# jgmarti84/radar-processor

Hardware: AMD Instinct MI355X
Metric: Mvoxels/s gridded (+ achieved HBM GB/s in roofline) (higher is better)
Workload: dtype f32

## Files before the change

### radar_processor_amd/csrc/rg_compact_layout.hpp

```cpp
#pragma once

#include <type_traits>

#include "rg_common.hpp"
#include "rg_row_phase.hpp"

using rg_u32x4 = unsigned __attribute__((ext_vector_type(4)));
__device__ rg_u32x4 rg_buffer_load_v4u32(__amdgpu_buffer_rsrc_t, int voffset, int soffset, int aux)
    __asm("llvm.amdgcn.raw.ptr.buffer.load.v4i32");

__device__ float rg_fmul_legacy(float, float) __asm("llvm.amdgcn.fmul.legacy");

namespace rgl {

struct ChunkGrid {
  long line_len;
  long lines_per_plane;
  long n_planes;
  unsigned nsx;
  unsigned nyg;
  unsigned rot_step;
  unsigned seg_base;
  unsigned seg_extra;
  unsigned grp0;
};

struct RowwiseColumns {
  const int32_t* order = nullptr;
  float* planes = nullptr;
  float* col_val = nullptr;
  int32_t* col_arg = nullptr;
  long n_xy = 0;
  unsigned n_cols = 0;
  int pieces = 1, keep_lo = 0, n_keep = 0, col_lo = 0, col_hi = 0;
};

struct RowwisePlanes : RowwiseColumns {
  float* col_min = nullptr;
  float* col_mean = nullptr;
  const int32_t* sel[RG_MAX_SEL_PLANES] = {};
  float* samples = nullptr;
  int n_sel = 0;
};

struct StreamArgs {
  const void* indptr;
  bool is_i64;
  const void* records;
  const int64_t* rec_ptr;
  int rec_order;
  unsigned w_base;
  const int64_t* dict_ptr;
  const int32_t* dict;
  long n_vox, n_pairs, line_len, lines_per_plane;
  const float* packed;
  int n_fields, stride;
  long n_gates;
  float fill;
  float* out;
  int window_cap;
  int lanes_hint;
  hipStream_t stream;
  int max_fields;
  bool need_out;
  bool need_packed;
  const uint16_t* row_end16 = nullptr;
};

}

namespace {

using rgl::ChunkGrid;
using rgl::StreamArgs;
using rgl::RowwiseColumns;
using rgl::RowwisePlanes;
using rg::f32x2;
using rg::f32x4;
using rsrc_t = __amdgpu_buffer_rsrc_t;
constexpr int kRsrcRaw32 = 0x00020000;

__device__ __forceinline__ rsrc_t make_rsrc(const void* base, long bytes) {
  const unsigned nb = bytes >= 0xFFFFFFFFL ? 0xFFFFFFFFu : bytes <= 0 ? 0u : (unsigned)bytes;
  return __builtin_amdgcn_make_buffer_rsrc(const_cast<void*>(base), 0, (int)nb, kRsrcRaw32);
}

constexpr int kH = RG_COMPACT_LINES;

__device__ __forceinline__ unsigned block_chunk(const ChunkGrid& g, unsigned bid) {
  const unsigned grp = bid / g.nsx;
  const unsigned col = bid - grp * g.nsx;
  const unsigned rot = col + ((grp + g.grp0) * g.rot_step) % g.nsx;
  return grp * g.nsx + (rot >= g.nsx ? rot - g.nsx : rot);
}

__host__ __device__ inline long chunk_count(const ChunkGrid& g) { return g.n_planes * (long)g.nyg * (long)g.nsx; }

struct Segment {
  long r0;
  long seg;
  int nrows;
};

__device__ __forceinline__ Segment chunk_segment(const ChunkGrid& g, unsigned chunk, int w) {
  const unsigned grp = chunk / g.nsx;
  const unsigned sx = chunk - grp * g.nsx;
  const unsigned plane = grp / g.nyg;
  const unsigned yg = grp - plane * g.nyg;
  const long y = (long)yg * kH + w;
  Segment s;
  if (y >= g.lines_per_plane) {
    s.r0 = 0;
    s.seg = 0;
    s.nrows = 0;
    return s;
  }
  s.seg = ((long)plane * g.lines_per_plane + y) * g.nsx + sx;
  const unsigned x0 = sx * g.seg_base + (sx < g.seg_extra ? sx : g.seg_extra);
  s.r0 = ((long)plane * g.lines_per_plane + y) * g.line_len + (long)x0;
  s.nrows = (int)(g.seg_base + (sx < g.seg_extra ? 1u : 0u));
  return s;
}

using rg::stride_for;

constexpr int kDenseMaxDict = RG_DENSE_MAX_DICT;
__host__ __device__ inline bool rec_is_dense(long nd_all) { return nd_all <= kDenseMaxDict; }
__host__ __device__ inline long rec_units(long n_rec, bool dense) { return dense ? (14 * n_rec + 15) >> 4 : n_rec; }

struct RecFields {
  unsigned wc[3];
  unsigned pos[3];
};

template <bool DENSE>
__device__ __forceinline__ RecFields rec_decode(const rg_u32x4& ld, unsigned par) {
  RecFields r;
  if constexpr (DENSE) {
    const unsigned sh = par << 4;
    const unsigned w2 = __builtin_amdgcn_alignbit(ld.w, ld.x, sh);
    r.wc[0] = ld.y;
    r.wc[1] = ld.z;
    r.wc[2] = w2;
    r.pos[0] = __builtin_amdgcn_ubfe(ld.w, sh, 11u);
    const unsigned p1h = __builtin_amdgcn_ubfe(ld.w, sh + 11u, 5u);
    r.pos[1] = __builtin_amdgcn_alignbit(p1h, ld.y, 26);
    r.pos[2] = __builtin_amdgcn_alignbit(w2 >> 26, ld.z, 26);
  } else {
    r.wc[0] = ld.x;
    r.wc[1] = ld.y;
    r.wc[2] = ld.z;
    r.pos[0] = ld.w & 0xFFFFu;
    r.pos[1] = ld.w >> 16;
    unsigned p2b = ld.y >> 26, p2c = ld.z >> 26;
    asm volatile("" : "+v"(p2b), "+v"(p2c));
    r.pos[2] = (p2c << 12) | ((p2b << 6) | (ld.x >> 26));
  }
  return r;
}

__device__ __forceinline__ void rec_encode_dense(const unsigned (&code)[3], const unsigned (&pos)[3], bool odd, unsigned short (&h)[7]) {
  const unsigned m1 = (code[0] & 0x3FFFFFFu) | ((pos[1] & 0x3Fu) << 26);
  const unsigned m2 = (code[1] & 0x3FFFFFFu) | ((pos[2] & 0x3Fu) << 26);
  const unsigned w2 = (code[2] & 0x3FFFFFFu) | (((pos[2] >> 6) & 0x1Fu) << 26);
  const unsigned short p = (unsigned short)((pos[0] & 0x7FFu) | (((pos[1] >> 6) & 0x1Fu) << 11));
  const unsigned short m1l = (unsigned short)m1, m1h = (unsigned short)(m1 >> 16), m2l = (unsigned short)m2,
                       m2h = (unsigned short)(m2 >> 16), w2h = (unsigned short)(w2 >> 16);
  h[0] = (unsigned short)w2;
  h[1] = odd ? m1l : w2h;
  h[2] = odd ? m1h : m1l;
  h[3] = odd ? m2l : m1h;
  h[4] = odd ? m2h : m2l;
  h[5] = odd ? w2h : m2h;
  h[6] = p;
}

bool make_chunk_grid(int64_t n_rows, int64_t line_len, int64_t lines_per_plane, ChunkGrid* cg) {
  if (line_len <= 0) line_len = n_rows > 0 ? n_rows : 1;
  if (n_rows % line_len != 0) return false;
  const long n_lines = n_rows / line_len;
  if (lines_per_plane <= 0) lines_per_plane = n_lines > 0 ? n_lines : 1;
  if (n_lines % lines_per_plane != 0) return false;
  cg->line_len = line_len;
  cg->lines_per_plane = lines_per_plane;
  cg->n_planes = n_lines / lines_per_plane;
  const long nsx = (line_len + 63) / 64, nyg = (lines_per_plane + kH - 1) / kH;
  if (nsx > 0x7FFFFFFFL || nyg > 0x7FFFFFFFL) return false;
  cg->nsx = (unsigned)nsx;
  cg->nyg = (unsigned)nyg;
  cg->seg_base = (unsigned)(line_len / nsx);
  cg->seg_extra = (unsigned)(line_len % nsx);
  cg->rot_step = RG_COMPACT_ROTATION;
  cg->grp0 = 0;
  return true;
}

inline int check_stream_args(const char* fn, const StreamArgs& a, ChunkGrid* cg) {
  RG_REQUIRE(a.rec_order == RG_REC_ORDER_SEGMENT || a.rec_order == RG_REC_ORDER_DISPATCH, RG_EINVAL,
             "%s: rec_order=%d is neither RG_REC_ORDER_SEGMENT nor RG_REC_ORDER_DISPATCH", fn, a.rec_order);
  RG_REQUIRE(a.n_fields >= 1 && a.n_fields <= a.max_fields, RG_EUNSUPPORTED, "%s: n_fields=%d not in 1..%d", fn, a.n_fields,
             a.max_fields);
  RG_REQUIRE(a.stride == stride_for(a.n_fields), RG_EINVAL, "%s: stride=%d, expected %d for %d fields", fn, a.stride,
             stride_for(a.n_fields), a.n_fields);
  RG_REQUIRE(a.indptr && a.dict_ptr && a.rec_ptr && (a.out || !a.need_out), RG_EINVAL, "%s: null indptr/dict_ptr/rec_ptr%s", fn,
             a.need_out ? "/out" : "");
  RG_REQUIRE(a.n_vox >= 0 && a.n_pairs >= 0, RG_EINVAL, "%s: negative size", fn);
  RG_REQUIRE(a.n_pairs == 0 || (a.records && a.dict && a.packed && a.n_gates > 0), RG_EINVAL,
             "%s: pairs present but records/dict/packed/n_gates missing", fn);
  RG_REQUIRE(!a.need_packed || (a.packed && a.n_gates > 0), RG_EINVAL, "%s: packed fields missing", fn);
  RG_REQUIRE(a.n_gates <= 0x7FFFFFFFL, RG_EUNSUPPORTED, "%s: n_gates exceeds int32 gate indices", fn);
  RG_REQUIRE(a.n_vox <= 0x3FFFFFFFFFL, RG_EUNSUPPORTED, "%s: n_vox too large for one launch", fn);
  RG_REQUIRE(a.window_cap >= 0 && a.window_cap <= RG_COMPACT_MAX_WINDOW, RG_EINVAL, "%s: window_cap %d outside 0..%d", fn,
             a.window_cap, RG_COMPACT_MAX_WINDOW);
  RG_REQUIRE(rg::aligned16(a.records), RG_EALIGN, "%s: records must be 16-byte aligned", fn);
  RG_REQUIRE(!a.need_packed || rg::aligned16(a.packed), RG_EALIGN, "%s: packed must be 16-byte aligned", fn);
  RG_REQUIRE((a.w_base & 0x3FFFFFFu) == 0, RG_EINVAL,
             "%s: w_base=0x%08x must have its low 26 bits clear (exponent a multiple of 8)", fn, a.w_base);
  RG_REQUIRE(a.lanes_hint == 0 || (a.lanes_hint >= 1 && a.lanes_hint <= 64 && (a.lanes_hint & (a.lanes_hint - 1)) == 0) ||
                 (a.lanes_hint > 70 && a.lanes_hint <= 99), RG_EINVAL,
             "%s: the lane split must be 0, a power of two up to 64, or 71..99", fn);
  if (a.n_vox == 0) return RG_OK;
  RG_REQUIRE(make_chunk_grid(a.n_vox, a.line_len, a.lines_per_plane, cg), RG_EINVAL,
             "%s: n_vox=%ld is not planes x lines_per_plane=%ld x line_len=%ld", fn, a.n_vox, a.lines_per_plane, a.line_len);
  RG_REQUIRE(chunk_count(*cg) <= 0x7FFFFFFFL, RG_EUNSUPPORTED, "%s: too many chunks for one launch", fn);
  return RG_OK;
}

template <int NF> struct RowwiseConfig;
template <> struct RowwiseConfig<1> { static constexpr int kpre = 3, target = 4; static constexpr bool regs = false; };
template <> struct RowwiseConfig<2> { static constexpr int kpre = 3, target = 4; static constexpr bool regs = false; };
template <> struct RowwiseConfig<3> { static constexpr int kpre = 3, target = 6; static constexpr bool regs = true; };
template <> struct RowwiseConfig<4> { static constexpr int kpre = 3, target = 8; static constexpr bool regs = true; };
template <> struct RowwiseConfig<5> { static constexpr int kpre = 3, target = 8; static constexpr bool regs = true; };
template <> struct RowwiseConfig<6> { static constexpr int kpre = 3, target = 8; static constexpr bool regs = true; };
template <> struct RowwiseConfig<7> { static constexpr int kpre = 3, target = 8; static constexpr bool regs = true; };
template <> struct RowwiseConfig<8> { static constexpr int kpre = 3, target = 12; static constexpr bool regs = true; };

template <int NF> constexpr bool rowwise_bytemask() { return NF >= 3; }
template <int NF> constexpr int rowwise_value_words() {
  return rowwise_bytemask<NF>() ? (NF <= 4 ? 4 : 8) : 2;
}
template <int NF> constexpr int rowwise_mask_words() { return !rowwise_bytemask<NF>() || NF == 3 ? 0 : NF == 4 ? 1 : 2; }
template <int NF> constexpr int rowwise_entry_words() { return rowwise_value_words<NF>() + rowwise_mask_words<NF>(); }


struct ColumnBest {
  float v;
  int idx;
};

__device__ __forceinline__ void column_max_step(ColumnBest& acc, float v, int z) {
  if (acc.idx < 0) {
    if (!isnan(v)) { acc.v = v; acc.idx = z; }
  } else {
    const bool keep = acc.v >= v || isnan(v);
    if (!keep) { acc.v = v; acc.idx = z; }
  }
}

__device__ __forceinline__ void column_min_step(float& acc, float v) {
  const bool keep = acc <= v || isnan(v);
  if (!keep) acc = v;
}

}

int rg_launch_tile_packed(const rgl::StreamArgs& a, const rgl::ChunkGrid& cg);
```

### radar_processor_amd/csrc/rg_csr_rowwise.hpp

```cpp
#pragma once

#include "rg_compact_layout.hpp"

namespace {

constexpr int kRowwiseChunksPerBlock = 1;

#define RG_ROWWISE_BOUNDS __launch_bounds__(64 * kH, (COLS == 2 ? (NF <= 2 ? 5 : 4) : (COLS == 0 && NF >= 4 && NF <= 6) ? 5 : 1))
template <typename IndT, int NF, int STRIDE, int COLS = 0, int REGS = -1>
__global__ RG_ROWWISE_BOUNDS void csr_compact_rowwise_kernel(
    const IndT* __restrict__ indptr, const int64_t* __restrict__ dict_ptr, const int32_t* __restrict__ dict, ChunkGrid cg,
    const float* __restrict__ packed, unsigned last_gate, float fill, int window_cap, long n_vox, float* __restrict__ out,
    const rg_u32x4* __restrict__ rec, const int64_t* __restrict__ rec_ptr, unsigned w_base, int lanes_hint,
    int rec_order, unsigned n_chunks, int chunks_per_block, const std::conditional_t<COLS == 2, RowwisePlanes, RowwiseColumns> cols,
    const uint16_t* __restrict__ row_end16) {
  static_assert(NF >= 1 && NF <= 8 && STRIDE == stride_for(NF), "passes of 1-8 fields");
  constexpr bool PLANES = COLS == 2;
  static_assert(!PLANES || NF <= 4, "the planes mode is the column mode of 1-4 fields");
  using Cfg = RowwiseConfig<NF>;
  constexpr int KPRE = Cfg::kpre;
  constexpr bool kByteMask = rowwise_bytemask<NF>();
  constexpr bool kRegs = REGS < 0 ? Cfg::regs : REGS != 0;
  constexpr bool kScatter = NF >= 5 && !COLS;
  constexpr int kFenceMinNF = 3;
  constexpr bool kPremask = NF == 1;
  extern __shared__ __attribute__((aligned(16))) float window[];
  constexpr int kVW = rowwise_value_words<NF>(), kMW = rowwise_mask_words<NF>();
#if defined(__HIP_DEVICE_COMPILE__) && !defined(__gfx950__)
#error "the byte masks assume v_cvt_pk_f32_fp8 decodes OCP e4m3 (0x38 = 1.0), as on gfx950"
#endif
  constexpr unsigned kMaskOne = 0x38u;
  (void)kMW;
  unsigned* const maskw = reinterpret_cast<unsigned*>(window + (size_t)(window_cap + 1) * kVW);
  __shared__ f32x2 rowacc_all[kRegs ? 1 : kH][kRegs ? 2 : 64 * NF];
  constexpr bool kStage = kScatter;
  __shared__ __attribute__((aligned(16))) float stage_all[kStage ? kH : 1][kStage ? 64 * 8 : 4];

  const int lane = threadIdx.x & 63;
  const int wv = __builtin_amdgcn_readfirstlane(threadIdx.x >> 6);
  f32x2* rowacc = rowacc_all[kRegs ? 0 : wv];
  float* const stage = stage_all[kStage ? wv : 0];
  unsigned wmask = 0x3FFFFFFu;
  asm volatile("" : "+v"(wmask));

  unsigned col_yg = 0, col_sx = 0, col_piece = 0;
  int col_z0 = 0;
  ColumnBest best[COLS ? NF : 1];
  float pmin[PLANES ? NF : 1], psum[PLANES ? NF : 1];
  int pcnt[PLANES ? NF : 1];
  if constexpr (PLANES) {
#pragma unroll
    for (int f = 0; f < NF; ++f) { pmin[f] = __builtin_nanf(""); psum[f] = 0.0f; pcnt[f] = 0; }
  }
  if constexpr (COLS) {
    const unsigned item = cols.order ? (unsigned)cols.order[blockIdx.x] : blockIdx.x;
    col_piece = item / cols.n_cols;
    const unsigned q = item - col_piece * cols.n_cols;
    col_yg = q / cg.nsx;
    const unsigned c = q - col_yg * cg.nsx;
    col_sx = c + (col_yg * cg.rot_step) % cg.nsx;
    col_sx = col_sx >= cg.nsx ? col_sx - cg.nsx : col_sx;
    col_z0 = (int)((long)col_piece * cg.n_planes / cols.pieces);
    chunks_per_block = (int)((long)(col_piece + 1) * cg.n_planes / cols.pieces) - col_z0;
#pragma unroll
    for (int f = 0; f < NF; ++f) { best[f].v = __builtin_nanf(""); best[f].idx = -1; }
  }
  long col_xy = 0;
  int col_nrows = 0;
  const int n_cb = COLS ? chunks_per_block : kRowwiseChunksPerBlock;
  for (int cb = 0; cb < n_cb; ++cb) {
  unsigned bid, chunk;
  if constexpr (COLS) {
    const unsigned grp = (unsigned)(col_z0 + cb) * cg.nyg + col_yg;
    chunk = grp * cg.nsx + col_sx;
    const unsigned shift = ((grp + cg.grp0) * cg.rot_step) % cg.nsx;
    bid = grp * cg.nsx + (col_sx >= shift ? col_sx - shift : col_sx + cg.nsx - shift);
  } else {
    bid = blockIdx.x * (unsigned)kRowwiseChunksPerBlock + (unsigned)cb;
    if (bid >= n_chunks) break;
    chunk = block_chunk(cg, bid);
  }
  if constexpr (!COLS) {
    if (rec_order == RG_REC_ORDER_DISPATCH && rec_ptr[(long)bid * kH] == rec_ptr[((long)bid + 1) * kH]) {
      const Segment se = chunk_segment(cg, chunk, wv);
      if (lane < se.nrows) {
#pragma unroll
        for (int f = 0; f < NF; ++f) out[(size_t)f * n_vox + se.r0 + lane] = fill;
      }
      continue;
    }
  }
  if (cb > 0) __syncthreads();
  float mine_p[NF], mine_w[NF];
#pragma unroll
  for (int f = 0; f < NF; ++f) mine_p[f] = mine_w[f] = 0.0f;

  const long d0 = dict_ptr[chunk];
  const int nd_all = (int)(dict_ptr[chunk + 1] - d0);
  const bool split = nd_all > 65536;
  const bool windowed = nd_all <= window_cap;

  const Segment sg = chunk_segment(cg, chunk, wv);
  const int nrows = sg.nrows;
  const long r0 = sg.r0;
  int span = 0, rs_o = 0, re_o = 0;
  unsigned e16 = RG_ROW_END16_WIDE;
  if (row_end16 && nrows) e16 = row_end16[r0 + (lane < nrows ? lane : nrows - 1)];
  if (__builtin_amdgcn_readlane((int)e16, 63) != (int)RG_ROW_END16_WIDE) {
    re_o = (int)e16;
    rs_o = __builtin_amdgcn_update_dpp(0, (int)e16, 0x138 , 0xF, 0xF, false);
    span = __builtin_amdgcn_readlane((int)e16, 63);
  } else if (nrows) {
    const long seg_b = (long)indptr[r0];
    span = (int)((long)indptr[r0 + nrows] - seg_b);
    rs_o = (int)((long)indptr[r0 + (lane < nrows ? lane : nrows)] - seg_b);
    re_o = (int)((long)indptr[r0 + (lane + 1 < nrows ? lane + 1 : nrows)] - seg_b);
  }
  long rec_b = 0, rec_n = 0;
  if (nrows) {
    const long slot = rec_order == RG_REC_ORDER_DISPATCH ? (long)bid * kH + wv : sg.seg;
    rec_b = rec_ptr[slot];
    rec_n = rec_ptr[slot + 1] - rec_b;
  }
  const rsrc_t rr = make_rsrc(rec + rec_b, rec_n * 16);
  const bool dense = rec_is_dense(nd_all);
  constexpr int kOutOfRange = 0x7FFFFFF0;

  int lgl;
  if (lanes_hint > 0 && lanes_hint <= 64) {
    lgl = 31 - __builtin_clz(lanes_hint);
  } else {
    const int target = lanes_hint > 70 ? lanes_hint - 70 : Cfg::target;
    const int mean_rec = nrows ? span / (3 * nrows) + 1 : 1;
    const int need = (mean_rec + target - 1) / target;
    lgl = need <= 1 ? 0 : 32 - __builtin_clz(need - 1);
  }
  lgl = __builtin_amdgcn_readfirstlane(lgl > 6 ? 6 : lgl);
  const int nl = 1 << lgl, rpr = 64 >> lgl;
  const int sub = lane & (nl - 1), rgrp = lane >> lgl;
  const int rounds = (nrows + rpr - 1) >> (6 - lgl);
  const unsigned q0_row = (unsigned)rs_o / 3u;
  const unsigned q1_row = re_o > rs_o ? ((unsigned)re_o + 2u) / 3u : q0_row;
  int trips_row = (int)((q1_row - q0_row + (unsigned)nl - 1u) >> lgl);
  for (int m = 1; m < rpr; m <<= 1) {
    const int o = __shfl_xor(trips_row, m, 64);
    trips_row = o > trips_row ? o : trips_row;
  }

  if (windowed) {
    constexpr int kFillBatch = 4;
    const int last_entry = nd_all > 0 ? nd_all - 1 : 0;
    const int32_t* __restrict__ cd = nd_all > 0 ? dict + d0 : (const int32_t*)dict_ptr;
    for (int i0 = threadIdx.x; i0 <= nd_all; i0 += 64 * kH * kFillBatch) {
      unsigned gate[kFillBatch];
#pragma unroll
      for (int u = 0; u < kFillBatch; ++u) {
        const int i = i0 + u * 64 * kH;
        gate[u] = (unsigned)cd[i < last_entry ? i : last_entry];
      }
      float v[kFillBatch][STRIDE];
#pragma unroll
      for (int u = 0; u < kFillBatch; ++u) rg::load_packed<STRIDE>(packed, gate[u] < last_gate ? gate[u] : last_gate, v[u]);
#pragma unroll
      for (int u = 0; u < kFillBatch; ++u) {
        const int i_raw = i0 + u * 64 * kH;
        const int i = i_raw < nd_all ? i_raw : nd_all;
        if (i_raw >= nd_all) {
#pragma unroll
          for (int s = 0; s < STRIDE; ++s) v[u][s] = __builtin_bit_cast(float, RG_EXCLUDED_BITS);
        }
        if constexpr (kByteMask) {
          unsigned m[2] = {0u, 0u};
          float vv[8] = {0.0f, 0.0f, 0.0f, 0.0f, 0.0f, 0.0f, 0.0f, 0.0f};
#pragma unroll
          for (int f = 0; f < NF; ++f) {
            const bool good = rg::f32_bits(v[u][f]) != RG_EXCLUDED_BITS;
            vv[f] = good ? v[u][f] : 0.0f;
            m[f >> 2] |= good ? (kMaskOne << (8 * (f & 3))) : 0u;
          }
          if constexpr (NF == 3) {
            reinterpret_cast<f32x4*>(window)[i] = (f32x4){vv[0], vv[1], vv[2], __builtin_bit_cast(float, m[0])};
          } else if constexpr (NF == 4) {
            reinterpret_cast<f32x4*>(window)[i] = (f32x4){vv[0], vv[1], vv[2], vv[3]};
            maskw[i] = m[0];
          } else {
            reinterpret_cast<f32x4*>(window)[2 * i] = (f32x4){vv[0], vv[1], vv[2], vv[3]};
            reinterpret_cast<f32x4*>(window)[2 * i + 1] = (f32x4){vv[4], vv[5], vv[6], vv[7]};
            reinterpret_cast<uint2*>(maskw)[i] = make_uint2(m[0], m[1]);
          }
        } else if constexpr (kPremask) {
          const bool good = rg::f32_bits(v[u][0]) != RG_EXCLUDED_BITS;
          reinterpret_cast<f32x2*>(window)[i] = good ? (f32x2){v[u][0], 1.0f} : (f32x2){0.0f, 0.0f};
        } else {
          reinterpret_cast<f32x2*>(window)[i] = (f32x2){v[u][0], v[u][1]};
        }
      }
    }
  }
  __syncthreads();

  struct Step {
    int lo0;
    unsigned len;
    int rem;
    int off0;
    int myrow, rho;
    int left;
    bool live;
  };
  auto setup = [&](auto dtag, int rho) -> Step {
    constexpr int rec_bytes = decltype(dtag)::value ? 14 : 16;
    Step r;
    r.rho = rho;
    r.myrow = rho * rpr + rgrp;
    r.live = r.myrow < nrows;
    const int qs = __shfl(rs_o, r.myrow & 63, 64);
    const int qe_row = __shfl(re_o, r.myrow & 63, 64);
    const int qe = r.live ? qe_row : qs;
    const int q0 = (int)((unsigned)qs / 3u);
    const int q1 = qe > qs ? (int)(((unsigned)qe + 2u) / 3u) : q0;
    const int q = q0 + sub;
    r.lo0 = qs - 3 * q;
    r.len = (unsigned)(qe - qs);
    r.rem = decltype(dtag)::value ? 2 * (q1 - q) + (q & 1) : q1 - q;
    r.off0 = q * rec_bytes;
    r.left = rho < rounds ? __builtin_amdgcn_readfirstlane(__shfl(trips_row, (rho * rpr) & 63, 64)) : 0;
    return r;
  };
  auto advance = [&](auto dtag, const Step& r) -> Step {
    constexpr int rec_bytes = decltype(dtag)::value ? 14 : 16;
    if (r.left > KPRE) {
      Step n = r;
      n.lo0 -= 3 * (KPRE << lgl);
      if constexpr (decltype(dtag)::value) n.rem = (n.rem - 2 * (KPRE << lgl)) ^ ((KPRE << lgl) & 1);
      else n.rem -= KPRE << lgl;
      n.off0 += rec_bytes * (KPRE << lgl);
      n.left -= KPRE;
      return n;
    }
    return setup(dtag, r.rho + 1);
  };
  auto issue = [&](auto dtag, const Step& r, rg_u32x4 (&regs)[KPRE]) {
    constexpr bool kDense = decltype(dtag)::value;
#pragma unroll
    for (int k = 0; k < KPRE; ++k) {
      const int off = kDense ? (r.off0 + 14 * (k << lgl)) & ~3 : r.off0 + 16 * (k << lgl);
      const bool has = kDense ? 2 * (k << lgl) + 1 < r.rem : (k << lgl) < r.rem;
      regs[k] = rg_buffer_load_v4u32(rr, has ? off : kOutOfRange, 0, 0);
    }
  };
  auto run = [&](auto wtag, auto dtag) {
    constexpr bool kWindowed = decltype(wtag)::value;
    constexpr bool kDense = decltype(dtag)::value;
    const int w_lo = !kWindowed && split ? dict[d0 + wv] : 0;
    const int w_hi = !kWindowed && split && wv + 1 < kH ? dict[d0 + wv + 1] : nd_all;
    const int nd_last = w_hi - w_lo > 0 ? w_hi - w_lo - 1 : 0;
    const int32_t* __restrict__ cdict = dict + d0 + w_lo;
    constexpr int KS = 2;
    constexpr int KSW = NF >= 5 ? 1 : KS;
    constexpr int NP2 = (NF + 1) / 2;
    float ap[kByteMask ? 1 : KS][kByteMask ? 1 : NF], aw[kByteMask ? 1 : KSW][kByteMask ? 1 : NF];
    f32x2 bp[kByteMask ? KS : 1][kByteMask ? NP2 : 1], bw[kByteMask ? KSW : 1][kByteMask ? NP2 : 1];
#pragma unroll
    for (int k = 0; k < (kByteMask ? 1 : KS); ++k) {
#pragma unroll
      for (int f = 0; f < (kByteMask ? 1 : NF); ++f) ap[k][f] = 0.0f;
    }
#pragma unroll
    for (int k = 0; k < (kByteMask ? 1 : KSW); ++k) {
#pragma unroll
      for (int f = 0; f < (kByteMask ? 1 : NF); ++f) aw[k][f] = 0.0f;
    }
#pragma unroll
    for (int k = 0; k < (kByteMask ? KS : 1); ++k) {
#pragma unroll
      for (int j = 0; j < (kByteMask ? NP2 : 1); ++j) bp[k][j] = (f32x2)(0.0f);
    }
#pragma unroll
    for (int k = 0; k < (kByteMask ? KSW : 1); ++k) {
#pragma unroll
      for (int j = 0; j < (kByteMask ? NP2 : 1); ++j) bw[k][j] = (f32x2)(0.0f);
    }
    auto addp = [&](int k, int f, float x) {
      if constexpr (kByteMask) bp[k][f >> 1][f & 1] += x; else ap[k][f] += x;
    };
    auto addw = [&](int k, int f, float x) {
      if constexpr (kByteMask) bw[k][f >> 1][f & 1] += x; else aw[k][f] += x;
    };
    auto fence_sums = [&](int kp, int kw) {
      if constexpr (kByteMask) {
#pragma unroll
        for (int j = 0; j < NP2; ++j) asm volatile("" : "+v"(bp[kp][j]), "+v"(bw[kw][j]) : : "memory");
      } else {
#pragma unroll
        for (int f = 0; f < NF; ++f) asm volatile("" : "+v"(ap[kp][f]), "+v"(aw[kw][f]) : : "memory");
      }
    };
    auto consume = [&](const Step& r, const rg_u32x4& q4, int k) {
      const int hi = r.lo0 + (int)r.len;
      float w[3];
      int pos[3];
      const RecFields rf = rec_decode<kDense>(q4, !kDense ? 0u : (k & 1) ? (unsigned)r.rem ^ (unsigned)(k << lgl) : (unsigned)r.rem);
#pragma unroll
      for (int i = 0; i < 3; ++i) {
        w[i] = __builtin_bit_cast(float, (rf.wc[i] & wmask) | w_base);
        pos[i] = (int)rf.pos[i];
      }
#pragma unroll
      for (int i = 0; i < 3; ++i) {
        const bool mine = 3 * (k << lgl) + i < hi && (k > 0 || i == 2 || r.lo0 <= i);
        const int p = kWindowed ? pos[i] : (pos[i] < nd_last ? pos[i] : nd_last);
        float v[STRIDE];
        if constexpr (kWindowed) {
          const int e = mine ? p : nd_all;
          __builtin_assume((unsigned)e <= 65536u);
          if constexpr (kByteMask) {
            float vv[8];
            unsigned m[2] = {0u, 0u};
            if constexpr (NF <= 4) {
              const f32x4 x = reinterpret_cast<const f32x4*>(window)[e];
              vv[0] = x.x; vv[1] = x.y; vv[2] = x.z; vv[3] = x.w;
              m[0] = NF == 3 ? rg::f32_bits(x.w) : maskw[e];
            } else {
              const f32x4 x = reinterpret_cast<const f32x4*>(window)[2 * e], y = reinterpret_cast<const f32x4*>(window)[2 * e + 1];
              vv[0] = x.x; vv[1] = x.y; vv[2] = x.z; vv[3] = x.w; vv[4] = y.x; vv[5] = y.y; vv[6] = y.z; vv[7] = y.w;
              const uint2 mm = reinterpret_cast<const uint2*>(maskw)[e];
              m[0] = mm.x; m[1] = mm.y;
            }
            using g2_t = decltype(__builtin_amdgcn_cvt_pk_f32_fp8(0, false));
            const g2_t a = __builtin_amdgcn_cvt_pk_f32_fp8((int)m[0], false), b = __builtin_amdgcn_cvt_pk_f32_fp8((int)m[0], true);
            const g2_t c = __builtin_amdgcn_cvt_pk_f32_fp8((int)m[1], false), d = __builtin_amdgcn_cvt_pk_f32_fp8((int)m[1], true);
            const f32x2 g2[4] = {(f32x2){a[0], a[1]}, (f32x2){b[0], b[1]}, (f32x2){c[0], c[1]}, (f32x2){d[0], d[1]}};
            const f32x2 w2 = (f32x2){w[i], w[i]};
#pragma unroll
            for (int j = 0; j < NP2; ++j) {
              const f32x2 prod = w2 * (f32x2){vv[2 * j], vv[2 * j + 1]};
              bp[k % KS][j] += prod;
              bw[k % KSW][j] = __builtin_elementwise_fma(w2, g2[j], bw[k % KSW][j]);
            }
            if constexpr (NF >= kFenceMinNF) fence_sums(k % KS, k % KSW);
            continue;
          } else if constexpr (kPremask) {
            const f32x2 term = (f32x2){w[i], w[i]} * reinterpret_cast<const f32x2*>(window)[e];
            ap[k % KS][0] += term.x;
            aw[k % KSW][0] += term.y;
            continue;
          } else {
            const f32x2 x = reinterpret_cast<const f32x2*>(window)[e];
            v[0] = x.x; v[1] = x.y;
          }
        } else {
          const unsigned g0 = (unsigned)cdict[p];
          rg::load_packed<STRIDE>(packed, g0 < last_gate ? g0 : last_gate, v);
          if (!mine) {
#pragma unroll
            for (int s = 0; s < STRIDE; ++s) v[s] = __builtin_bit_cast(float, RG_EXCLUDED_BITS);
          }
        }
#pragma unroll
        for (int f = 0; f < NF; ++f) {
          const bool good = rg::f32_bits(v[f]) != RG_EXCLUDED_BITS;
          const float wf = good ? w[i] : 0.0f;
          addp(k % KS, f, rg_fmul_legacy(wf, v[f]));
          addw(k % KSW, f, wf);
        }
        if constexpr (NF >= kFenceMinNF) fence_sums(k % KS, k % KSW);
      }
    };
    auto process = [&](const Step& r, const rg_u32x4 (&regs)[KPRE], bool last) {
#pragma unroll
      for (int k = 0; k < KPRE; ++k) {
        if (k < r.left) consume(r, regs[k], k);
      }
      if (!last) return;
      float sv[2 * NF];
#pragma unroll
      for (int f = 0; f < NF; ++f) {
        float sp, sw;
        if constexpr (kByteMask) {
          sp = bp[0][f >> 1][f & 1];
          sw = bw[0][f >> 1][f & 1];
#pragma unroll
          for (int k = 1; k < KS; ++k) sp += bp[k][f >> 1][f & 1];
#pragma unroll
          for (int k = 1; k < KSW; ++k) sw += bw[k][f >> 1][f & 1];
        } else {
          sp = ap[0][f];
          sw = aw[0][f];
          ap[0][f] = aw[0][f] = 0.0f;
#pragma unroll
          for (int k = 1; k < KS; ++k) {
            sp += ap[k][f];
            ap[k][f] = 0.0f;
          }
#pragma unroll
          for (int k = 1; k < KSW; ++k) {
            sw += aw[k][f];
            aw[k][f] = 0.0f;
          }
        }
        sv[2 * f] = sp;
        sv[2 * f + 1] = sw;
      }
      if constexpr (kByteMask) {
#pragma unroll
        for (int k = 0; k < KS; ++k) {
#pragma unroll
          for (int j = 0; j < NP2; ++j) bp[k][j] = (f32x2)(0.0f);
        }
#pragma unroll
        for (int k = 0; k < KSW; ++k) {
#pragma unroll
          for (int j = 0; j < NP2; ++j) bw[k][j] = (f32x2)(0.0f);
        }
      }
      rg::butterfly<2 * NF>(sv, nl);
      if constexpr (kScatter) {
        constexpr int NP = NF <= 2 ? 2 : NF <= 4 ? 4 : 8, LGP = NF <= 2 ? 1 : NF <= 4 ? 2 : 3;
        float p[NP], w[NP];
#pragma unroll
        for (int f = 0; f < NP; ++f) {
          p[f] = f < NF ? sv[2 * (f < NF ? f : 0)] : 0.0f;
          w[f] = f < NF ? sv[2 * (f < NF ? f : 0) + 1] : 0.0f;
        }
        const int stages = lgl < LGP ? lgl : LGP;
#pragma unroll
        for (int st = 0; st < LGP; ++st) {
          if (st < stages) {
            const bool bit = ((sub >> st) & 1) != 0;
#pragma unroll
            for (int i = 0; i < (NP >> (st + 1)); ++i) {
              p[i] = bit ? p[2 * i + 1] : p[2 * i];
              w[i] = bit ? w[2 * i + 1] : w[2 * i];
            }
          }
        }
        const int lp = 1 << stages;
        const int f0 = sub & (lp - 1);
        const bool owner = r.live && (sub >> stages) == 0;
        float* dst = out + ((size_t)f0 * n_vox + r0 + r.myrow);
        const size_t step_f = (size_t)lp * n_vox;
#pragma unroll
        for (int j = 0; j < NP; ++j) {
          if (j < (NP >> stages)) {
            if constexpr (kStage) {
              if (owner && f0 + j * lp < NF) stage[r.myrow * 8 + f0 + j * lp] = w[j] > 0.0f ? p[j] / w[j] : fill;
            } else {
              if (owner && f0 + j * lp < NF) dst[j * step_f] = w[j] > 0.0f ? p[j] / w[j] : fill;
            }
          }
        }
      } else if constexpr (kRegs) {
        const int first = r.myrow - rgrp;
        const bool take = lane >= first && lane < first + rpr;
        const int src = ((lane - first) << lgl) & 63;
#pragma unroll
        for (int f = 0; f < NF; ++f) {
          const float gp = __shfl(sv[2 * f], src, 64), gw = __shfl(sv[2 * f + 1], src, 64);
          mine_p[f] = take ? gp : mine_p[f];
          mine_w[f] = take ? gw : mine_w[f];
        }
      } else if (r.live && sub == 0) {
#pragma unroll
        for (int f = 0; f < NF; ++f) rowacc[r.myrow * NF + f] = (f32x2){sv[2 * f], sv[2 * f + 1]};
      }
    };

    rg_u32x4 regs_a[KPRE], regs_b[KPRE];
    Step sa = setup(dtag, 0), sb;
    issue(dtag, sa, regs_a);
    for (;;) {
      sb = advance(dtag, sa);
      issue(dtag, sb, regs_b);
      process(sa, regs_a, sb.rho != sa.rho);
      if (sb.rho >= rounds) break;
      sa = advance(dtag, sb);
      issue(dtag, sa, regs_a);
      process(sb, regs_b, sa.rho != sb.rho);
      if (sa.rho >= rounds) break;
    }
  };
  if (span > 0) {
    if (dense) {
      if (windowed) run(std::true_type{}, std::true_type{}); else run(std::false_type{}, std::true_type{});
    } else {
      if (windowed) run(std::true_type{}, std::false_type{}); else run(std::false_type{}, std::false_type{});
    }
  }
  int psel[PLANES ? RG_MAX_SEL_PLANES : 1];
  unsigned pxy = 0;
  if constexpr (PLANES) {
    pxy = (unsigned)(r0 - (long)(col_z0 + cb) * cols.n_xy) + (unsigned)lane;
#pragma unroll
    for (int s = 0; s < RG_MAX_SEL_PLANES; ++s) psel[s] = (s < cols.n_sel && lane < nrows) ? cols.sel[s][pxy] : RG_PPI_SEL_NONE;
  }
  __builtin_amdgcn_fence(__ATOMIC_RELEASE, "wavefront");
  __builtin_amdgcn_wave_barrier();
  __builtin_amdgcn_fence(__ATOMIC_ACQUIRE, "wavefront");

  if constexpr (kStage) {
    if (span > 0 && lane < nrows) {
      int sl = lane;
      asm volatile("" : "+v"(sl));
      const f32x4 lo = reinterpret_cast<const f32x4*>(stage)[2 * sl], hi = reinterpret_cast<const f32x4*>(stage)[2 * sl + 1];
      const float vals[8] = {lo.x, lo.y, lo.z, lo.w, hi.x, hi.y, hi.z, hi.w};
#pragma unroll
      for (int f = 0; f < NF; ++f) out[(size_t)f * n_vox + r0 + lane] = vals[f];
    }
  }
  if (lane < nrows && !(kScatter && span > 0)) {
#pragma unroll
    for (int f = 0; f < NF; ++f) {
      f32x2 s = (f32x2)(0.0f);
      if constexpr (kRegs) s = (f32x2){mine_p[f], mine_w[f]};
      else if (span > 0) s = rowacc[lane * NF + f];
      if constexpr (COLS) {
        const float val = s.y > 0.0f ? (float)((double)s.x / (double)s.y) : fill;
        const int z = col_z0 + cb;
        if (out) out[(size_t)f * n_vox + r0 + lane] = val;
        if (cols.planes && z >= cols.keep_lo && z < cols.keep_lo + cols.n_keep)
          cols.planes[((size_t)f * cols.n_keep + (z - cols.keep_lo)) * cols.n_xy + (r0 - (long)z * cols.n_xy) + lane] = val;
        if (cols.col_val && z >= cols.col_lo && z <= cols.col_hi) column_max_step(best[f], val, z);
        if constexpr (PLANES) {
          if (z >= cols.col_lo && z <= cols.col_hi) {
            if (cols.col_min) column_min_step(pmin[f], val);
            if (cols.col_mean) {
              const bool nan = isnan(val);
              psum[f] = __fadd_rn(psum[f], nan ? 0.0f : val);
              pcnt[f] += nan ? 0 : 1;
            }
          }
#pragma unroll
          for (int s = 0; s < RG_MAX_SEL_PLANES; ++s) {
            if (s < cols.n_sel) {
              float* const smp = cols.samples + ((size_t)(f * cols.n_sel + s) * 2) * cols.n_xy;
              if (z == (psel[s] & 0xFFFF)) smp[pxy] = val;
              if (z == (int)((unsigned)psel[s] >> 16)) smp[cols.n_xy + pxy] = val;
            }
          }
        }
      } else {
        out[(size_t)f * n_vox + r0 + lane] = s.y > 0.0f ? (float)((double)s.x / (double)s.y) : fill;
      }
    }
  }
  if constexpr (COLS) {
    col_nrows = nrows;
    col_xy = r0 - (long)(col_z0 + cb) * cols.n_xy + lane;
    if constexpr (!kRegs) {
      __builtin_amdgcn_fence(__ATOMIC_RELEASE, "wavefront");
      __builtin_amdgcn_wave_barrier();
      __builtin_amdgcn_fence(__ATOMIC_ACQUIRE, "wavefront");
    }
  }
  }
  if constexpr (PLANES) {
    if (lane < col_nrows) {
#pragma unroll
      for (int f = 0; f < NF; ++f) {
        const size_t o = ((size_t)col_piece * NF + f) * cols.n_xy + col_xy;
        if (cols.col_val) {
          cols.col_val[o] = best[f].v;
          if (cols.col_arg) cols.col_arg[o] = best[f].idx;
        }
        if (cols.col_min) cols.col_min[o] = pmin[f];
        if (cols.col_mean) cols.col_mean[o] = (float)((double)psum[f] / (double)pcnt[f]);
      }
    }
  } else if constexpr (COLS) {
    if (cols.col_val && lane < col_nrows) {
#pragma unroll
      for (int f = 0; f < NF; ++f) {
        const size_t o = ((size_t)col_piece * NF + f) * cols.n_xy + col_xy;
        cols.col_val[o] = best[f].v;
        if (cols.col_arg) cols.col_arg[o] = best[f].idx;
      }
    }
  }
}

template <typename IndT, int NF, int COLS, int REGS, typename Cols>
int launch_rowwise(const char* fn, const StreamArgs& a, const ChunkGrid& cg, long static_lds, dim3 grid, int chunks_per_block,
                   const Cols& cols) {
  constexpr int WS = rowwise_entry_words<NF>();
  const long room = (65536 - static_lds - 256) / (4 * WS) - 1;
  const int window_cap = a.window_cap > room ? (int)room : a.window_cap;
  hipLaunchKernelGGL((csr_compact_rowwise_kernel<IndT, NF, stride_for(NF), COLS, REGS>), grid, dim3(64 * kH),
                     ((size_t)(window_cap + 1) * WS * sizeof(float) + 15) / 16 * 16, a.stream, static_cast<const IndT*>(a.indptr),
                     a.dict_ptr, a.dict, cg, a.packed, (unsigned)(a.n_gates - 1), a.fill, window_cap, a.n_vox, a.out,
                     static_cast<const rg_u32x4*>(a.records), a.rec_ptr, a.w_base, a.lanes_hint, a.rec_order,
                     (unsigned)chunk_count(cg), chunks_per_block, cols, a.row_end16);
  return rg::check_launch(fn);
}

}
```

Measured before the change: 22830.

## Precompute per-row record descriptors and use DPP butterfly in rowwise CSR kernel

Each lane now precomputes a packed row descriptor (byte offset plus first-position and end bounds) once per row. Rows are set up with ds_bpermute and readlane instead of shuffles and per-step divisions. The dense decode shift is derived from the byte offset, which removes the parity/remainder bookkeeping, and bounds checks use a single hi comparison. The reduction uses a DPP-based butterfly with an SGPR-held lane count, plus a register-pinned sentinel, to cut shuffle and scalar overhead in the inner loop, at the cost of more intricate index arithmetic.

```diff
diff --git a/radar_processor_amd/csrc/rg_compact_layout.hpp b/radar_processor_amd/csrc/rg_compact_layout.hpp
--- a/radar_processor_amd/csrc/rg_compact_layout.hpp
+++ b/radar_processor_amd/csrc/rg_compact_layout.hpp
@@ -134,10 +134,9 @@
 };
 
 template <bool DENSE>
-__device__ __forceinline__ RecFields rec_decode(const rg_u32x4& ld, unsigned par) {
+__device__ __forceinline__ RecFields rec_decode_at(const rg_u32x4& ld, unsigned sh) {
   RecFields r;
   if constexpr (DENSE) {
-    const unsigned sh = par << 4;
     const unsigned w2 = __builtin_amdgcn_alignbit(ld.w, ld.x, sh);
     r.wc[0] = ld.y;
     r.wc[1] = ld.z;
@@ -159,6 +158,11 @@
   return r;
 }
 
+template <bool DENSE>
+__device__ __forceinline__ RecFields rec_decode(const rg_u32x4& ld, unsigned par) {
+  return rec_decode_at<DENSE>(ld, par << 4);
+}
+
 __device__ __forceinline__ void rec_encode_dense(const unsigned (&code)[3], const unsigned (&pos)[3], bool odd, unsigned short (&h)[7]) {
   const unsigned m1 = (code[0] & 0x3FFFFFFu) | ((pos[1] & 0x3Fu) << 26);
   const unsigned m2 = (code[1] & 0x3FFFFFFu) | ((pos[2] & 0x3Fu) << 26);
@@ -173,6 +177,35 @@
   h[4] = odd ? m2h : m2l;
   h[5] = odd ? w2h : m2h;
   h[6] = p;
+}
+
+struct RowDesc {
+  unsigned boff;
+  unsigned pack;
+};
+
+__host__ __device__ inline int row_records(int rs, int re) {
+  return re > rs ? (int)(((unsigned)re + 2u) / 3u - (unsigned)rs / 3u) : 0;
+}
+__host__ __device__ inline RowDesc row_desc_make(int rs, int re, int rec_bytes) {
+  const unsigned q0 = (unsigned)rs / 3u;
+  const unsigned fp = (unsigned)rs - 3u * q0;
+  RowDesc d;
+  d.boff = q0 * (unsigned)rec_bytes;
+  d.pack = re > rs ? (fp + (unsigned)(re - rs)) | (fp << 30) : 0u;
+  return d;
+}
+
+struct LaneStart {
+  int lo0, hi, off0;
+};
+template <bool DENSE>
+__host__ __device__ inline LaneStart row_desc_lane(const RowDesc& d, int sub) {
+  LaneStart s;
+  s.lo0 = (int)(d.pack >> 30) - 3 * sub;
+  s.hi = (int)(d.pack & 0x3FFFFFFFu) - 3 * sub;
+  s.off0 = (int)d.boff + sub * (DENSE ? 14 : 16);
+  return s;
 }
 
 bool make_chunk_grid(int64_t n_rows, int64_t line_len, int64_t lines_per_plane, ChunkGrid* cg) {
diff --git a/radar_processor_amd/csrc/rg_csr_rowwise.hpp b/radar_processor_amd/csrc/rg_csr_rowwise.hpp
--- a/radar_processor_amd/csrc/rg_csr_rowwise.hpp
+++ b/radar_processor_amd/csrc/rg_csr_rowwise.hpp
@@ -5,6 +5,29 @@
 namespace {
 
 constexpr int kRowwiseChunksPerBlock = 1;
+
+template <int N>
+__device__ __forceinline__ void rowwise_butterfly(float (&v)[N], int nsub) {
+  auto stage = [&](auto ctrl) {
+#pragma unroll
+    for (int i = 0; i < N; ++i) {
+      v[i] += rg::dpp_f32<decltype(ctrl)::value>(v[i]);
+      asm volatile("" : "+v"(v[i]));
+    }
+  };
+  if (nsub > 1) stage(rg::int_c<0xB1>{});
+  if (nsub > 2) stage(rg::int_c<0x4E>{});
+  if (nsub > 4) stage(rg::int_c<0x141>{});
+  if (nsub > 8) stage(rg::int_c<0x140>{});
+  if (nsub > 16) {
+#pragma unroll
+    for (int i = 0; i < N; ++i) v[i] += __shfl_xor(v[i], 16, 64);
+  }
+  if (nsub > 32) {
+#pragma unroll
+    for (int i = 0; i < N; ++i) v[i] += __shfl_xor(v[i], 32, 64);
+  }
+}
 
 #define RG_ROWWISE_BOUNDS __launch_bounds__(64 * kH, (COLS == 2 ? (NF <= 2 ? 5 : 4) : (COLS == 0 && NF >= 4 && NF <= 6) ? 5 : 1))
 template <typename IndT, int NF, int STRIDE, int COLS = 0, int REGS = -1>
@@ -139,9 +162,8 @@
   const int nl = 1 << lgl, rpr = 64 >> lgl;
   const int sub = lane & (nl - 1), rgrp = lane >> lgl;
   const int rounds = (nrows + rpr - 1) >> (6 - lgl);
-  const unsigned q0_row = (unsigned)rs_o / 3u;
-  const unsigned q1_row = re_o > rs_o ? ((unsigned)re_o + 2u) / 3u : q0_row;
-  int trips_row = (int)((q1_row - q0_row + (unsigned)nl - 1u) >> lgl);
+  const RowDesc desc = row_desc_make(rs_o, re_o, dense ? 14 : 16);
+  int trips_row = (row_records(rs_o, re_o) + nl - 1) >> lgl;
   for (int m = 1; m < rpr; m <<= 1) {
     const int o = __shfl_xor(trips_row, m, 64);
     trips_row = o > trips_row ? o : trips_row;
@@ -201,30 +223,28 @@
 
   struct Step {
     int lo0;
-    unsigned len;
-    int rem;
+    int hi;
     int off0;
     int myrow, rho;
     int left;
     bool live;
   };
   auto setup = [&](auto dtag, int rho) -> Step {
-    constexpr int rec_bytes = decltype(dtag)::value ? 14 : 16;
     Step r;
     r.rho = rho;
     r.myrow = rho * rpr + rgrp;
     r.live = r.myrow < nrows;
-    const int qs = __shfl(rs_o, r.myrow & 63, 64);
-    const int qe_row = __shfl(re_o, r.myrow & 63, 64);
-    const int qe = r.live ? qe_row : qs;
-    const int q0 = (int)((unsigned)qs / 3u);
-    const int q1 = qe > qs ? (int)(((unsigned)qe + 2u) / 3u) : q0;
-    const int q = q0 + sub;
-    r.lo0 = qs - 3 * q;
-    r.len = (unsigned)(qe - qs);
-    r.rem = decltype(dtag)::value ? 2 * (q1 - q) + (q & 1) : q1 - q;
-    r.off0 = q * rec_bytes;
-    r.left = rho < rounds ? __builtin_amdgcn_readfirstlane(__shfl(trips_row, (rho * rpr) & 63, 64)) : 0;
+    RowDesc d = {0u, 0u};
+    r.left = 0;
+    if (rho < rounds) {
+      d.boff = (unsigned)__builtin_amdgcn_ds_bpermute(r.myrow << 2, (int)desc.boff);
+      d.pack = (unsigned)__builtin_amdgcn_ds_bpermute(r.myrow << 2, (int)desc.pack);
+      r.left = __builtin_amdgcn_readlane(trips_row, rho * rpr);
+    }
+    const LaneStart s = row_desc_lane<decltype(dtag)::value>(d, sub);
+    r.lo0 = s.lo0;
+    r.hi = s.hi;
+    r.off0 = s.off0;
     return r;
   };
   auto advance = [&](auto dtag, const Step& r) -> Step {
@@ -232,8 +252,7 @@
     if (r.left > KPRE) {
       Step n = r;
       n.lo0 -= 3 * (KPRE << lgl);
-      if constexpr (decltype(dtag)::value) n.rem = (n.rem - 2 * (KPRE << lgl)) ^ ((KPRE << lgl) & 1);
-      else n.rem -= KPRE << lgl;
+      n.hi -= 3 * (KPRE << lgl);
       n.off0 += rec_bytes * (KPRE << lgl);
       n.left -= KPRE;
       return n;
@@ -245,7 +264,7 @@
 #pragma unroll
     for (int k = 0; k < KPRE; ++k) {
       const int off = kDense ? (r.off0 + 14 * (k << lgl)) & ~3 : r.off0 + 16 * (k << lgl);
-      const bool has = kDense ? 2 * (k << lgl) + 1 < r.rem : (k << lgl) < r.rem;
+      const bool has = 3 * (k << lgl) < r.hi;
       regs[k] = rg_buffer_load_v4u32(rr, has ? off : kOutOfRange, 0, 0);
     }
   };
@@ -256,6 +275,8 @@
     const int w_hi = !kWindowed && split && wv + 1 < kH ? dict[d0 + wv + 1] : nd_all;
     const int nd_last = w_hi - w_lo > 0 ? w_hi - w_lo - 1 : 0;
     const int32_t* __restrict__ cdict = dict + d0 + w_lo;
+    int sentinel = nd_all;
+    if constexpr (kWindowed) asm volatile("" : "+v"(sentinel));
     constexpr int KS = 2;
     constexpr int KSW = NF >= 5 ? 1 : KS;
     constexpr int NP2 = (NF + 1) / 2;
@@ -297,10 +318,10 @@
       }
     };
     auto consume = [&](const Step& r, const rg_u32x4& q4, int k) {
-      const int hi = r.lo0 + (int)r.len;
+      const int hi = r.hi;
       float w[3];
       int pos[3];
-      const RecFields rf = rec_decode<kDense>(q4, !kDense ? 0u : (k & 1) ? (unsigned)r.rem ^ (unsigned)(k << lgl) : (unsigned)r.rem);
+      const RecFields rf = rec_decode_at<kDense>(q4, !kDense ? 0u : (unsigned)((k & 1) ? r.off0 + 14 * (k << lgl) : r.off0) << 3);
 #pragma unroll
       for (int i = 0; i < 3; ++i) {
         w[i] = __builtin_bit_cast(float, (rf.wc[i] & wmask) | w_base);
@@ -312,7 +333,7 @@
         const int p = kWindowed ? pos[i] : (pos[i] < nd_last ? pos[i] : nd_last);
         float v[STRIDE];
         if constexpr (kWindowed) {
-          const int e = mine ? p : nd_all;
+          const int e = mine ? p : sentinel;
           __builtin_assume((unsigned)e <= 65536u);
           if constexpr (kByteMask) {
             float vv[8];
@@ -414,7 +435,9 @@
           for (int j = 0; j < NP2; ++j) bw[k][j] = (f32x2)(0.0f);
         }
       }
-      rg::butterfly<2 * NF>(sv, nl);
+      int nsub = nl;
+      asm volatile("" : "+s"(nsub));
+      rowwise_butterfly<2 * NF>(sv, nsub);
       if constexpr (kScatter) {
         constexpr int NP = NF <= 2 ? 2 : NF <= 4 ? 4 : 8, LGP = NF <= 2 ? 1 : NF <= 4 ? 2 : 3;
         float p[NP], w[NP];
```

Result: no change. 22980 (median of 6 runs) (+0.6%).
